# supranational/sppark

Hardware: AMD Instinct MI355X
Metric: MSM points/sec (BLS12-381 G1, 2^26 points) (higher is better)
Workload: dtype u32

## Files before the change

### sppark_amd/csrc/msm/msm_driver.hpp

```cpp
#pragma once
#include "msm_kernels.hpp"
#include "msm_coop_kernels.hpp"
#include "msm_plan.hpp"
#include "../ec/jacobian_host.hpp"
#include "../util/runtime.hpp"
#include <algorithm>
#include <cmath>
#include <map>
#include <mutex>
#include <vector>

namespace sppark_amd {

template<class FD, class FH, class FRp>
class msm_t {
public:
    typedef FD fp_d;
    static constexpr bool G2_COOP_BUILT = field_is_internal<FD>::value && !field_is_montx<FD>::value;
    typedef mont_dev<FRp> fr_d;
    typedef FH fp_h;
    typedef typename xyzz_dev<fp_d>::mem_t bucket_t;
    typedef jacobian_host<fp_h> point_t;
    static constexpr int STD_WORDS = sizeof(FH) / 4;
    static constexpr size_t FP_BYTES = sizeof(FH);
// ... 248 lines not shown
    {
        if (tune.wbits) return std::min(26u, std::max(8u, tune.wbits));
        unsigned w = 0; double best = 0;
        for (unsigned c = 8; c <= 26; c++) {
            const double cost = (double)((FRp::NBITS - 1) / c + 1) * (double)np + 3.0 * (double)((size_t)1 << (c - 1));
            if (w == 0 || cost < best) { best = cost; w = c; }
        }
        return w;
    }
    void preload(const void* points, size_t np, size_t ffi_affine_sz, bool fixed_base = false)
    {
        HIP_OK(hipSetDevice(gpu->hip_id));
        HIP_OK(hipStreamSynchronize(stream));
        join_default_stream();
        if (np != 0 && (points == nullptr || ffi_affine_sz < 2 * FP_BYTES || np > (1u << 31))) HIP_OK(hipErrorInvalidValue);
        if (np != 0 && fixed_base && !MONTX) HIP_OK(hipErrorNotSupported);
        if (np != 0 && fixed_base && (tune.wbits || np >= FIXED_BASE_MIN)
            && (size_t)((FRp::NBITS - 1) / fixed_base_width(np) + 1) * np >= ((size_t)1 << 31)) HIP_OK(hipErrorInvalidValue);
        if (pre_points) { HIP_OK(hipFree(pre_points)); pre_points = nullptr; pre_n = pre_stride = 0; }
        pre_fb_wbits = pre_fb_nwins = 0;
        if (np == 0) return;
        if (fixed_base && !MONTX) HIP_OK(hipErrorNotSupported);
        if (fixed_base && !tune.wbits && np < FIXED_BASE_MIN) fixed_base = false;
        unsigned fb_w = 0, fb_nw = 1;
        if (fixed_base) {
            fb_w = fixed_base_width(np);
            fb_nw = (FRp::NBITS - 1) / fb_w + 1;
            fb_w = FRp::NBITS / fb_nw + (FRp::NBITS % fb_nw ? 1 : 0);
            if ((size_t)fb_nw * np >= ((size_t)1 << 31)) HIP_OK(hipErrorInvalidValue);
        }
        if (points == nullptr || ffi_affine_sz < 2 * FP_BYTES || np > (1u << 31)) HIP_OK(hipErrorInvalidValue);
        struct dev_buf {
            unsigned char* p = nullptr;
            ~dev_buf() { if (p) (void)hipFree(p); }
        } staging;
        try {
            if constexpr (INTERNAL) {
                const unsigned char* src = (const unsigned char*)points;
                if (!is_device_pointer(points)) {
                    HIP_OK(hipMalloc((void**)&staging.p, np * ffi_affine_sz));
                    HIP_OK(hipMemcpyAsync(staging.p, points, np * ffi_affine_sz, hipMemcpyHostToDevice, stream));
                    src = staging.p;
                }
                HIP_OK(dev_scratch_pool::malloc_or_drain((void**)&pre_points, (size_t)fb_nw * np * conv_stride()));
                launch_convert(pre_points, src, (unsigned)np, ffi_affine_sz);
                if constexpr (MONTX) if (fixed_base) {
                    hipLaunchKernelGGL(k_fixed_base_table<fp_d>, dim3((unsigned)((np + 255) / 256)), dim3(256), 0, stream,
                                       pre_points, (unsigned)np, fb_nw, (unsigned)FRp::NBITS);
                    HIP_OK(hipGetLastError());
                }
            } else {
                HIP_OK(hipMalloc((void**)&pre_points, np * ffi_affine_sz));
                HIP_OK(hipMemcpyAsync(pre_points, points, np * ffi_affine_sz,
                                      is_device_pointer(points) ? hipMemcpyDeviceToDevice : hipMemcpyHostToDevice, stream));
            }
            HIP_OK(hipStreamSynchronize(stream));
        } catch (...) {
            if (pre_points) { (void)hipFree(pre_points); pre_points = nullptr; }
            throw;
        }
        pre_n = np; pre_stride = ffi_affine_sz;
        if (fixed_base) { pre_fb_wbits = fb_w; pre_fb_nwins = fb_nw; }
    }
    unsigned fixed_base_windows() const { return pre_fb_nwins; }
    size_t preloaded() const { return pre_n; }

private:
    void launch_convert(unsigned char* dst, const unsigned char* src, unsigned n, size_t stride, hipStream_t on = nullptr)
    {
        if constexpr (INTERNAL) {
            if (on == nullptr) on = stream;
            unsigned grid = (n + 255) / 256;
            if constexpr (MONTX) {
                if ((stride == 2 * FP_BYTES || stride == 2 * FP_BYTES + 8) && ((size_t)src & 15) == 0 && tune.join != 6) {
                    if (stride == 2 * FP_BYTES) hipLaunchKernelGGL((k_convert_points_staged<fp_d, false>), dim3(grid), dim3(256), 0, on, dst, src, n);
                    else                        hipLaunchKernelGGL((k_convert_points_staged<fp_d, true>), dim3(grid), dim3(256), 0, on, dst, src, n);
                    HIP_OK(hipGetLastError());
                    return;
                }
            }
            if (stride > 2 * FP_BYTES) hipLaunchKernelGGL((k_convert_points<fp_d, true>), dim3(grid), dim3(256), 0, on, dst, src, n, (unsigned)stride);
            else                       hipLaunchKernelGGL((k_convert_points<fp_d, false>), dim3(grid), dim3(256), 0, on, dst, src, n, (unsigned)stride);
            HIP_OK(hipGetLastError());
        }
    }

    size_t choose_chunk(size_t n, size_t stage_per_point) const
    {
        size_t chunk = n;
        if (tune.chunk) chunk = std::min(n, std::max<size_t>(tune.chunk, 1));
        else if (stage_per_point && n > ((size_t)1 << 21)) {
            chunk = std::min<size_t>(std::max<size_t>(n / 4, (size_t)1 << 20), (size_t)1 << 24);
        }
        auto need = [&](size_t c) {
            return make_layout(make_plan(c, FRp::NBITS, tune), true).total + 2 * c * stage_per_point + 1024;
        };
        size_t limit = tune.max_scratch;
        if (!limit) {
            const bool blob_ok = make_layout(make_plan(chunk, FRp::NBITS, tune), true).total <= blob_sz;
            const bool stage_ok = stage_per_point == 0 || 2 * (chunk * stage_per_point + 512) <= stage_sz;
            if (blob_ok && stage_ok) return chunk;
            size_t free_b = 0, total_b = 0;
            if (hipMemGetInfo(&free_b, &total_b) != hipSuccess) { (void)hipGetLastError(); return chunk; }
            limit = free_b - (free_b >> 5) + blob_sz + stage_sz;
        }
        while (need(chunk) > limit && chunk > 4096) chunk = (chunk + 1) / 2;
        return chunk;
    }

    std::vector<size_t> chunk_bounds(size_t n, size_t chunk) const
    {
        std::vector<size_t> b{0};
        for (size_t lo = chunk; lo < n; lo += chunk) b.push_back(lo);
        b.push_back(n);
        return b;
    }

    void sort_group(hipStream_t ss, const msm_plan& p, const layout& l, unsigned b, unsigned w0, unsigned wn,
                    const u32* d_scalars, bool mont, unsigned fb_n = 0, unsigned fb_nwins = 0)
    {
        u32* digits = (u32*)(blob + l.digits[b]);
        u32* sorted = (u32*)(blob + l.sorted[b]);
        u32* H = (u32*)(blob + l.H[b]);
        u32* tot = (u32*)(blob + l.tot[b]);
        u32* off = (u32*)(blob + l.off[b]);
        void* partA = blob + l.partA[b];
        u32* offA = (u32*)(blob + l.offA[b]);
        const bool packed = p.IB != 0;
        unsigned ngp = 1; while (ngp < p.NG) ngp <<= 1;
        const partA_fmt fmt{H, p.IB, p.SH, ngp, p.nslabs};
        const unsigned nlong = p.nbits % p.nwins, sf = nlong == 0 ? wn : (nlong > w0 ? std::min(wn, nlong - w0) : 0u);
        if (fb_n) {
            unsigned grid = std::min<unsigned>((fb_n + 255) / 256, 256 * 16);
            hipLaunchKernelGGL(k_breakdown<fr_d>, dim3(grid), dim3(256), 0, ss,
                               digits, d_scalars, fb_n, fb_nwins, (unsigned)FRp::NBITS, (int)mont, 0u, fb_nwins);
        } else {
            unsigned grid = std::min<unsigned>((p.n + 255) / 256, 256 * 16);
            hipLaunchKernelGGL(k_breakdown<fr_d>, dim3(grid), dim3(256), 0, ss,
                               digits, d_scalars, p.n, p.nwins, p.nbits, (int)mont, w0, wn);
        }
        HIP_OK(hipGetLastError());
        size_t ldsA = (size_t)p.NA * 4, ldsB = ((size_t)1 << p.LB) * 4 + SORT_NT * 4 + (size_t)SORTB_STAGE * 4 + PARTA_MAX_GROUPS * 4;
        if (ldsA > 65536) { lds_attr((const void*)k_histA, ldsA); lds_attr(packed ? (const void*)k_scatterA<true> : (const void*)k_scatterA<false>, ldsA); }
        if (ldsB > 65536) lds_attr(packed ? (const void*)k_sortB<true> : (const void*)k_sortB<false>, ldsB);
        hipLaunchKernelGGL(k_histA, dim3(p.nslabs, wn), dim3(SORT_NT), ldsA, ss,
                           H, digits, p.n, p.nslabs, p.slab_sz, p.NA, p.LB, sf);
        HIP_OK(hipGetLastError());
        size_t na_total = (size_t)wn * p.NA;
        hipLaunchKernelGGL(k_scan_slabs, dim3((unsigned)((na_total + 255) / 256)), dim3(256), 0, ss,
                           H, tot, p.nslabs, p.NA, wn);
        HIP_OK(hipGetLastError());
        hipLaunchKernelGGL(k_scan_parts, dim3(wn), dim3(1024), 0, ss, offA, tot, p.NA);
        HIP_OK(hipGetLastError());
        if (p.NA <= SCATA_MAX_NA && p.LB < 16) {
            const size_t ldsS = scatterA_staged_lds(p.NA);
            lds_attr(packed ? (const void*)k_scatterA_staged<true> : (const void*)k_scatterA_staged<false>, ldsS);
            if (packed) hipLaunchKernelGGL(k_scatterA_staged<true>, dim3(p.nslabs, wn), dim3(SORT_NT), ldsS, ss,
                                           (u32*)partA, digits, H, offA, p.n, p.nslabs, p.slab_sz, p.NA, p.LB, sf, p.IB);
            else        hipLaunchKernelGGL(k_scatterA_staged<false>, dim3(p.nslabs, wn), dim3(SORT_NT), ldsS, ss,
                                           (uint2*)partA, digits, H, offA, p.n, p.nslabs, p.slab_sz, p.NA, p.LB, sf, p.IB);
        } else {
            if (packed) hipLaunchKernelGGL(k_scatterA<true>, dim3(p.nslabs, wn), dim3(SORT_NT), ldsA, ss,
                                           (u32*)partA, digits, H, offA, p.n, p.nslabs, p.slab_sz, p.NA, p.LB, sf, p.IB);
            else        hipLaunchKernelGGL(k_scatterA<false>, dim3(p.nslabs, wn), dim3(SORT_NT), ldsA, ss,
                                           (uint2*)partA, digits, H, offA, p.n, p.nslabs, p.slab_sz, p.NA, p.LB, sf, p.IB);
        }
        HIP_OK(hipGetLastError());
        const unsigned big = tune.big ? tune.big : p.big ? p.big : (1u << 18);
        u32* nbig = (u32*)(blob + l.bigl[b]); u32* blist = nbig + 1; u32* curB = (u32*)(blob + l.curB[b]);
        const bool may_be_big = p.n > big;
        if (may_be_big) HIP_OK(hipMemsetAsync(nbig, 0, 4, ss));
        if (packed) hipLaunchKernelGGL(k_sortB<true>, dim3(p.NA, wn), dim3(SORT_NT), ldsB, ss,
                                       sorted, off, (const u32*)partA, offA, p.n, p.NA, p.LB, sf, big, fmt);
        else        hipLaunchKernelGGL(k_sortB<false>, dim3(p.NA, wn), dim3(SORT_NT), ldsB, ss,
                                       sorted, off, (const uint2*)partA, offA, p.n, p.NA, p.LB, sf, big, fmt);
        HIP_OK(hipGetLastError());
        if (!may_be_big) return;
        hipLaunchKernelGGL(k_big_find, dim3((p.NA * wn + 255) / 256), dim3(256), 0, ss,
                           nbig, blist, off, offA, p.NA, p.LB, sf, wn, big);
        size_t ldsBig = ((size_t)1 << p.LB) * 4;
        const size_t avg = (size_t)p.n / p.NA;
        const unsigned split = avg > big / 2 ? (unsigned)std::min<size_t>(SORTB_SPLIT, avg / (BIG_STAGE / 2) + 1) : SORTB_SPLIT;
        if (packed) hipLaunchKernelGGL(k_big_hist<true>, dim3(1024), dim3(1024), ldsBig, ss, off, (const u32*)partA, offA, nbig, blist, p.n, p.NA, p.LB, sf, split);
        else        hipLaunchKernelGGL(k_big_hist<false>, dim3(1024), dim3(1024), ldsBig, ss, off, (const uint2*)partA, offA, nbig, blist, p.n, p.NA, p.LB, sf, split);
        hipLaunchKernelGGL(k_big_scan, dim3(p.NA > 64 && avg > big / 2 ? 1024 : 64), dim3(1024), 0, ss, off, curB, offA, nbig, blist, p.NA, p.LB, sf);
        const size_t ldsSc = big_scatter_lds(p.LB);
        if (ldsSc > 65536) lds_attr(packed ? (const void*)k_big_scatter<true> : (const void*)k_big_scatter<false>, ldsSc);
        if (packed) hipLaunchKernelGGL(k_big_scatter<true>, dim3(1024), dim3(1024), ldsSc, ss, sorted, curB, (const u32*)partA, offA, nbig, blist, p.n, p.NA, p.LB, sf, split, fmt);
        else        hipLaunchKernelGGL(k_big_scatter<false>, dim3(1024), dim3(1024), ldsSc, ss, sorted, curB, (const uint2*)partA, offA, nbig, blist, p.n, p.NA, p.LB, sf, split, fmt);
        HIP_OK(hipGetLastError());
    }

    void enqueue(const msm_plan& p, const layout& l, const unsigned char* d_points, size_t stride, bool preconverted,
                 const u32* d_scalars, bool mont, std_bucket_t* h_out, bool first_timed, unsigned fb_n = 0, unsigned fb_nwins = 0,
                 bool redo = false, bool may_defer = false)
    {
        const bool flagged = !preconverted && stride > 2 * FP_BYTES;
        const bool multi = p.G > 1;
        if (multi) need_aux();
        if (timing && first_timed && !redo) { need_tev(2 + 2 * p.G); HIP_OK(hipEventRecord(tev[0], stream)); }
        if (multi) {
            HIP_OK(hipEventRecord(ev_fork, stream));
            HIP_OK(hipStreamWaitEvent(aux, ev_fork, 0));
        }
        bucket_t* buckets = (bucket_t*)(blob + l.buckets);
        u32* keyA = (u32*)(blob + l.keyA); bucket_t* ptA = (bucket_t*)(blob + l.ptA);
        u32* keyB = (u32*)(blob + l.keyB); bucket_t* ptB = (bucket_t*)(blob + l.ptB);
        if (multi && !redo) HIP_OK(hipMemsetAsync(buckets, 0, (size_t)p.nwins * p.NB * sizeof(bucket_t), stream));

        for (unsigned g = 0; g < p.G && !redo; g++, gseq++) {
            const unsigned b = multi ? (gseq & 1) : 0, w0 = g * p.wpg, wn = std::min(p.wpg, p.nwins - w0);
            if (g == 0) {
                sort_group(stream, p, l, b, w0, wn, d_scalars, mont, fb_n, fb_nwins);
                if (INTERNAL && !preconverted) {
                    launch_convert(blob + l.conv, d_points, p.n, stride);
                    d_points = blob + l.conv;
                }
            } else {
                if (gseq >= 2) HIP_OK(hipStreamWaitEvent(aux, ev_accdone[b], 0));
                sort_group(aux, p, l, b, w0, wn, d_scalars, mont);
                HIP_OK(hipEventRecord(ev_sorted[b], aux));
                HIP_OK(hipStreamWaitEvent(stream, ev_sorted[b], 0));
            }
            if (timing && first_timed) HIP_OK(hipEventRecord(tev[2 + 2 * g], stream));
            {
                const u32* sorted = (const u32*)(blob + l.sorted[b]);
                const u32* off = (const u32*)(blob + l.off[b]);
                dim3 grid((p.chunks_per_win + 255) / 256, wn);
                bool by_pairs = false;
                if constexpr (G2_COOP_BUILT) {
                    if (tune.g2_coop == 1 || (tune.g2_coop == 0 && fp_d::NL >= 14)) {
                        by_pairs = true;
                        dim3 grid2((p.chunks_per_win + 63) / 64, wn);
                        hipLaunchKernelGGL((k_accumulate_g2c<fp_d>), grid2, dim3(G2C_NT), 0, stream,
                                           buckets, keyA, ptA, d_points, (unsigned)stride, sorted, off,
                                           p.n, p.NB, p.L, p.chunks_per_win, w0);
                    }
                }
                if (by_pairs) {}
                else if (flagged)
                    hipLaunchKernelGGL((k_accumulate<fp_d, true>), grid, dim3(256), 0, stream,
                                       buckets, keyA, ptA, d_points, (unsigned)stride, sorted, off,
                                       p.n, p.NB, p.L, p.chunks_per_win, w0);
                else
                    hipLaunchKernelGGL((k_accumulate<fp_d, false>), grid, dim3(256), 0, stream,
                                       buckets, keyA, ptA, d_points, (unsigned)stride, sorted, off,
                                       p.n, p.NB, p.L, p.chunks_per_win, w0);
                HIP_OK(hipGetLastError());
            }
            if (timing && first_timed) HIP_OK(hipEventRecord(tev[3 + 2 * g], stream));
            if (multi) HIP_OK(hipEventRecord(ev_accdone[b], stream));
        }

        const unsigned piece_cm = may_defer ? piece_tree_cmax(p, multi, fb_n) : 0;
        piece_pending = false;
        bool small_sums = false;
        if constexpr (MONTX)
            small_sums = !multi && fb_n == 0 && p.NB <= SMALL_SUMS_MAX_NB && p.NB >= 2 && tune.K1 == 0 && tune.top == 0 && tune.K == 0
                         && tune.join != 3 && tune.join != 4;
        bool flag_with_sums = false;
        if constexpr (MONTX) flag_with_sums = small_sums && (piece_cm != 0 || redo);
        if (flag_with_sums && !d_pflag) {
            HIP_OK(hipMalloc((void**)&d_pflag, 64));
            HIP_OK(hipMemsetAsync(d_pflag, 0, 64, stream));
        }
        if (piece_cm && !redo) {
            u32* flag = flag_with_sums ? d_pflag : (u32*)(blob + l.flag);
            if (!flag_with_sums) HIP_OK(hipMemsetAsync(flag, 0, 4, stream));
            const u32* off = (const u32*)(blob + l.off[0]);
            unsigned t_fused = ~0u;
            if constexpr (MONTX) if (tune.join != 4 && tune.join != 8)
                t_fused = piece_tail_t0((size_t)p.nwins * p.NB, piece_cm, tune.join >= 16 ? (size_t)1 << (tune.join - 16) : PIECE_FUSE_MAX);
            for (unsigned t = 0; (piece_cm >> (t + 1)) >= 1; t++) {
                const unsigned last = (piece_cm >> (t + 2)) == 0;
                const size_t nthr = (size_t)p.nwins * p.NB * (piece_cm >> (t + 1));
                if constexpr (MONTX) if (t == t_fused) {
                    const unsigned lgGB = piece_tail_lgGB(piece_cm, t);
                    const size_t nwg = (((size_t)p.nwins * p.NB) + ((size_t)1 << lgGB) - 1) >> lgGB;
                    hipLaunchKernelGGL(k_piece_tail_coop<fp_d>, dim3((unsigned)nwg), dim3(COOP_NT), 0, stream,
                                       buckets, keyA, ptA, off, p.NB, p.L, p.chunks_per_win, p.nwins, piece_cm, t, lgGB, flag);
                    HIP_OK(hipGetLastError());
                    break;
                }
                bool coop = false;
                if constexpr (MONTX) coop = nthr <= COOP_LEVEL_MAX && tune.join != 4;
                if constexpr (MONTX) {
                    if (coop) hipLaunchKernelGGL(k_piece_level_coop<fp_d>, dim3((unsigned)((nthr + 63) / 64)), dim3(COOP_NT), 0, stream,
                                                 buckets, keyA, ptA, off, p.NB, p.L, p.chunks_per_win, p.nwins, piece_cm, t, last, flag);
                }
                if (!coop) hipLaunchKernelGGL(k_piece_level<fp_d>, dim3((unsigned)((nthr + 255) / 256)), dim3(256), 0, stream,
                                              buckets, keyA, ptA, off, p.NB, p.L, p.chunks_per_win, p.nwins, piece_cm, t, last, flag);
                HIP_OK(hipGetLastError());
            }
            if (!h_flag) HIP_OK(hipHostMalloc((void**)&h_flag, 64, hipHostMallocDefault));
            if (!flag_with_sums) HIP_OK(hipMemcpyAsync(h_flag, flag, 4, hipMemcpyDeviceToHost, stream));
            h_flag_cur = flag_with_sums ? reinterpret_cast<const u32*>(h_out + p.nwins) : h_flag;
            piece_pending = true;
        }
        if (!piece_pending) {
            size_t nrec = (size_t)2 * p.nwins * p.chunks_per_win;
            u32* ik = keyA; bucket_t* ip = ptA; u32* ok = keyB; bucket_t* op = ptB;
            const u32* skip = nullptr;
            if (tune.join != 1 && !redo && (size_t)p.n / p.NB <= (size_t)4 * p.L) {
                u32* keyC = (u32*)(blob + l.keyC); u32* flag = (u32*)(blob + l.flag);
                HIP_OK(hipMemsetAsync(flag, 0, 4, stream));
                const size_t nthr = nrec / 2 + 1;
                hipLaunchKernelGGL(k_join_runs<fp_d>, dim3((unsigned)((nthr + 255) / 256)), dim3(256), 0, stream,
                                   buckets, keyC, keyA, ptA, (unsigned)nrec, flag);
                HIP_OK(hipGetLastError());
                ik = keyC; skip = flag;
            }
            bool coop_tree = false;
            if constexpr (MONTX) coop_tree = tune.join != 4 && tune.join != 2;
// ... 381 lines not shown
```

### sppark_amd/csrc/msm/msm_sort_kernels.hpp

```cpp
#pragma once
#include "../ff/mont_dev.hpp"
#include "msm_sort_records.hpp"

namespace sppark_amd {

static constexpr unsigned SORT_NT = 1024;
#define SORT_VGPRS 32
static constexpr int SORTB_UNROLL = 4;
static constexpr int SORTB_PER = 18;
static constexpr unsigned SORTB_STAGE = SORTB_PER * SORT_NT;

__host__ __device__ inline unsigned window_lb(unsigned LB, unsigned w, unsigned short_from)
{   return (w >= short_from && LB) ? LB - 1 : LB;   }

SPPARK_DEVFN u32 block_scan_excl(u32 s, u32* wsum, u32* total)
{
    const unsigned lane = threadIdx.x & 63, wave = threadIdx.x >> 6;
    u32 incl = s;
    #pragma unroll
    for (int dlt = 1; dlt < 64; dlt <<= 1) { u32 v = __shfl_up(incl, dlt); if (lane >= (unsigned)dlt) incl += v; }
    if (lane == 63) wsum[wave] = incl;
    __syncthreads();
    u32 wv = lane < 16 ? wsum[lane] : 0, before = lane < wave ? wv : 0, tot = wv;
    #pragma unroll
    for (int m = 1; m < 16; m <<= 1) { before += __shfl_xor(before, m); tot += __shfl_xor(tot, m); }
    before = __shfl(before, 0); *total = __shfl(tot, 0);
    __syncthreads();
    return before + incl - s;
}

__global__ __launch_bounds__(SORT_NT) __attribute__((amdgpu_num_vgpr(SORT_VGPRS)))
void k_histA(u32* __restrict__ H, const u32* __restrict__ digits, unsigned n,
             unsigned nslabs, unsigned slab_sz, unsigned NA, unsigned LBL, unsigned short_from)
{
    extern __shared__ u32 lds_cnt[];
    const unsigned slab = blockIdx.x, w = blockIdx.y, LB = window_lb(LBL, w, short_from);
    for (unsigned b = threadIdx.x; b < NA; b += blockDim.x) lds_cnt[b] = 0;
    __syncthreads();

    const unsigned lo = slab * slab_sz, hi = min(n, lo + slab_sz);
    const u32* dig = digits + (size_t)w * n;
    for (unsigned i = lo + threadIdx.x; i < hi; i += 4 * blockDim.x) {
        u32 d[4];
        #pragma unroll
        for (int u = 0; u < 4; u++) { unsigned j = i + u * blockDim.x; d[u] = j < hi ? dig[j] : 0; }
        #pragma unroll
        for (int u = 0; u < 4; u++) if (d[u]) atomicAdd(&lds_cnt[((d[u] & 0x7fffffffu) - 1) >> LB], 1u);
    }
    __syncthreads();

    u32* out = H + ((size_t)w * nslabs + slab) * NA;
    for (unsigned b = threadIdx.x; b < NA; b += blockDim.x) out[b] = lds_cnt[b];
}

__global__ __launch_bounds__(256)
void k_scan_slabs(u32* __restrict__ H, u32* __restrict__ tot, unsigned nslabs, unsigned NA, unsigned nwins)
{
    const size_t id = (size_t)blockIdx.x * 256 + threadIdx.x;
    if (id >= (size_t)nwins * NA) return;
    const unsigned w = id / NA, b = id % NA;
    u32 run = 0;
    for (unsigned s = 0; s < nslabs; s++) {
        u32* p = H + ((size_t)w * nslabs + s) * NA + b;
        u32 t = *p; *p = run; run += t;
    }
    tot[id] = run;
}

__global__ __launch_bounds__(1024)
void k_scan_parts(u32* __restrict__ offA, const u32* __restrict__ tot, unsigned NA)
{
    __shared__ u32 part[1024];
    const unsigned w = blockIdx.x, tid = threadIdx.x;
    const unsigned per = (NA + 1023) / 1024;
    const unsigned lo = min(NA, tid * per), hi = min(NA, lo + per);
    const u32* t = tot + (size_t)w * NA;
    u32 sum = 0;
    for (unsigned b = lo; b < hi; b++) sum += t[b];
    part[tid] = sum;
    __syncthreads();
    for (unsigned d = 1; d < 1024; d <<= 1) {
        u32 v = tid >= d ? part[tid - d] : 0;
        __syncthreads();
        part[tid] += v;
        __syncthreads();
    }
    u32 run = part[tid] - sum;
    u32* o = offA + (size_t)w * (NA + 1);
    for (unsigned b = lo; b < hi; b++) { o[b] = run; run += t[b]; }
    if (tid == 1023) o[NA] = part[1023];
}

template<bool PK>
__global__ __launch_bounds__(SORT_NT) __attribute__((amdgpu_num_vgpr(SORT_VGPRS)))
void k_scatterA(typename recA<PK>::type* __restrict__ partA, const u32* __restrict__ digits,
                const u32* __restrict__ H, const u32* __restrict__ offA,
                unsigned n, unsigned nslabs, unsigned slab_sz, unsigned NA, unsigned LBL, unsigned short_from, unsigned IB)
{
    extern __shared__ u32 lds_cur[];
    const unsigned slab = blockIdx.x, w = blockIdx.y, LB = window_lb(LBL, w, short_from);
    const u32* h = H + ((size_t)w * nslabs + slab) * NA;
    const u32* o = offA + (size_t)w * (NA + 1);
    for (unsigned b = threadIdx.x; b < NA; b += blockDim.x) lds_cur[b] = h[b] + o[b];
    __syncthreads();

    const unsigned lo = slab * slab_sz, hi = min(n, lo + slab_sz);
    const u32* dig = digits + (size_t)w * n;
    typename recA<PK>::type* dst = partA + (size_t)w * n;
    const u32 lomask = (1u << LB) - 1;
    for (unsigned i = lo + threadIdx.x; i < hi; i += 4 * blockDim.x) {
        u32 d[4];
        #pragma unroll
        for (int u = 0; u < 4; u++) { unsigned j = i + u * blockDim.x; d[u] = j < hi ? dig[j] : 0; }
        #pragma unroll
        for (int u = 0; u < 4; u++) {
            if (d[u]) {
                u32 k = (d[u] & 0x7fffffffu) - 1;
                u32 pos = atomicAdd(&lds_cur[k >> LB], 1u);
                dst[pos] = recA<PK>::make((i + u * blockDim.x) | (d[u] & 0x80000000u), k & lomask, LBL, IB);
            }
        }
    }
}

static constexpr int SCATA_PER = 14;
static constexpr unsigned SCATA_TILE = SCATA_PER * SORT_NT;
static constexpr unsigned SCATA_MAX_NA = 4 * SORT_NT;
static inline size_t scatterA_staged_lds(unsigned NA) { return (size_t)NA * 8 + 64 + (size_t)SCATA_TILE * 8; }

SPPARK_DEVFN void wait_vmem()
{
#if defined(__HIP_DEVICE_COMPILE__)
    __builtin_amdgcn_s_waitcnt(0x0f70);
#endif
}
SPPARK_DEVFN void lds_barrier()
{
#if defined(__HIP_DEVICE_COMPILE__)
    asm volatile("s_waitcnt lgkmcnt(0)\n\ts_barrier" ::: "memory");
#endif
}

template<bool PK>
__global__ __launch_bounds__(SORT_NT)
void k_scatterA_staged(typename recA<PK>::type* __restrict__ partA, const u32* __restrict__ digits,
                       const u32* __restrict__ H, const u32* __restrict__ offA,
                       unsigned n, unsigned nslabs, unsigned slab_sz, unsigned NA, unsigned LBL, unsigned short_from, unsigned IB)
{
    extern __shared__ u32 lds_sa[];
    constexpr unsigned NT = SORT_NT;
    u32* cnt = lds_sa;
    u32* G = cnt + NA;
    u32* wsum = G + NA;
    uint2* stage = reinterpret_cast<uint2*>(wsum + 16);
    const unsigned slab = blockIdx.x, w = blockIdx.y, tid = threadIdx.x, lane = tid & 63, wave = tid >> 6;
    const unsigned LB = window_lb(LBL, w, short_from);
    const u32* h = H + ((size_t)w * nslabs + slab) * NA;
    const u32* o = offA + (size_t)w * (NA + 1);
    u32 cur[4];
    #pragma unroll
    for (int i = 0; i < 4; i++) { unsigned b = 4 * tid + i; cur[i] = b < NA ? h[b] + o[b] : 0; if (b < NA) cnt[b] = 0; }

    const unsigned lo = slab * slab_sz, hi = min(n, lo + slab_sz);
    const u32* dig = digits + (size_t)w * n;
    typename recA<PK>::type* dst = partA + (size_t)w * n;
    const u32 lomask = (1u << LB) - 1;
    u32 d[SCATA_PER], dn[SCATA_PER];
    #pragma unroll
    for (int u = 0; u < SCATA_PER; u++) { unsigned j = lo + u * NT + tid; dn[u] = j < hi ? dig[j] : 0; }
    __syncthreads();

    wait_vmem();
    #pragma unroll
    for (int u = 0; u < SCATA_PER; u++) d[u] = dn[u];
    for (unsigned t0 = lo; t0 < hi; t0 += SCATA_TILE) {
        #pragma unroll
        for (int u = 0; u < SCATA_PER; u++) { unsigned j = t0 + SCATA_TILE + u * NT + tid; dn[u] = j < hi ? dig[j] : 0; }
        #pragma unroll
        for (int u = 0; u < SCATA_PER; u++) if (d[u]) atomicAdd(&cnt[((d[u] & 0x7fffffffu) - 1) >> LB], 1u);
        lds_barrier();
        u32 c[4], s = 0;
        #pragma unroll
        for (int i = 0; i < 4; i++) { unsigned b = 4 * tid + i; c[i] = b < NA ? cnt[b] : 0; s += c[i]; }
        u32 incl = s;
        #pragma unroll
        for (int dlt = 1; dlt < 64; dlt <<= 1) { u32 v = __shfl_up(incl, dlt); if (lane >= (unsigned)dlt) incl += v; }
        if (lane == 63) wsum[wave] = incl;
        lds_barrier();
        u32 wv = lane < 16 ? wsum[lane] : 0, before = lane < wave ? wv : 0, total = wv;
        #pragma unroll
        for (int m = 1; m < 16; m <<= 1) { before += __shfl_xor(before, m); total += __shfl_xor(total, m); }
        before = __shfl(before, 0); total = __shfl(total, 0);
        u32 run = before + incl - s;
        #pragma unroll
        for (int i = 0; i < 4; i++) {
            unsigned b = 4 * tid + i;
            if (b < NA) { cnt[b] = run; G[b] = cur[i] - run; }
            cur[i] += c[i]; run += c[i];
        }
        lds_barrier();
        #pragma unroll
        for (int u = 0; u < SCATA_PER; u++) {
            if (d[u]) {
                u32 k = (d[u] & 0x7fffffffu) - 1, p = k >> LB;
                u32 pos = atomicAdd(&cnt[p], 1u);
                stage[pos] = make_uint2((t0 + u * NT + tid) | (d[u] & 0x80000000u), (p << 16) | (k & lomask));
            }
        }
        lds_barrier();
        wait_vmem();
        #pragma unroll
        for (int u = 0; u < SCATA_PER; u++) d[u] = dn[u];
        #pragma unroll
        for (int i = 0; i < 4; i++) { unsigned b = 4 * tid + i; if (b < NA) cnt[b] = 0; }
        #pragma unroll
        for (int u = 0; u < SCATA_PER; u++) {
            unsigned e = u * NT + tid;
            if (e < total) { uint2 v = stage[e]; dst[G[v.y >> 16] + e] = recA<PK>::make(v.x, v.y & 0xffffu, LBL, IB); }
        }
        lds_barrier();
    }
}

template<bool PK>
__global__ __launch_bounds__(SORT_NT) __attribute__((amdgpu_num_vgpr(64)))
void k_sortB(u32* __restrict__ sorted, u32* __restrict__ off, const typename recA<PK>::type* __restrict__ partA,
             const u32* __restrict__ offA, unsigned n, unsigned NA, unsigned LBL, unsigned short_from, unsigned big, partA_fmt fmt)
{
    extern __shared__ u32 lds[];
    typedef typename recA<PK>::type rec_t;
    constexpr unsigned NT = SORT_NT;
    const unsigned LB = window_lb(LBL, blockIdx.y, short_from);
    const size_t NB = (size_t)NA << LBL;
    const unsigned NL = 1u << LB;
    const u32 kmask = (1u << LBL) - 1;
    u32* cnt = lds;
    u32* part = lds + NL;
    u32* stage = part + NT;
    u32* bnd = stage + SORTB_STAGE;
    const unsigned khi = blockIdx.x, w = blockIdx.y, tid = threadIdx.x;
    const u32* oA = offA + (size_t)w * (NA + 1);
    const unsigned begin = oA[khi], end = oA[khi + 1];
    const rec_t* src = partA + (size_t)w * n;
    if (end - begin > big) {
        if (khi == NA - 1 && tid == 0) off[(size_t)w * (NB + 1) + NB] = end;
        if (LB != LBL) for (unsigned b = tid; b < NL; b += NT) off[(size_t)w * (NB + 1) + ((size_t)(NA + khi) << LB) + b] = oA[NA];
        return;
    }
    if (LB != LBL) for (unsigned b = tid; b < NL; b += NT) off[(size_t)w * (NB + 1) + ((size_t)(NA + khi) << LB) + b] = oA[NA];

    const bool in_regs = end - begin <= SORTB_STAGE;
    rec_t rr[SORTB_PER];
    for (unsigned b = tid; b < NL; b += NT) cnt[b] = 0;
    if (PK) partA_bounds(bnd, fmt, w, khi, NA, tid);
    __syncthreads();
    if (in_regs) {
        #pragma unroll
        for (int u = 0; u < SORTB_PER; u++) {
            unsigned j = begin + tid + u * NT;
            if (j < end) rr[u] = src[j];
        }
        #pragma unroll
        for (int u = 0; u < SORTB_PER; u++) if (begin + tid + u * NT < end) atomicAdd(&cnt[recA<PK>::key(rr[u], kmask)], 1u);
    } else {
        for (unsigned i = begin + tid; i < end; i += SORTB_UNROLL * NT) {
            rec_t r[SORTB_UNROLL];
            #pragma unroll
            for (int u = 0; u < SORTB_UNROLL; u++) { unsigned j = i + u * NT; if (j < end) r[u] = src[j]; }
            #pragma unroll
            for (int u = 0; u < SORTB_UNROLL; u++) if (i + u * NT < end) atomicAdd(&cnt[recA<PK>::key(r[u], kmask)], 1u);
        }
    }
    __syncthreads();

    const unsigned per = (NL + NT - 1) / NT;
    const unsigned lo = min(NL, tid * per), hi = min(NL, lo + per);
    u32 sum = 0;
    #pragma unroll 1
    for (unsigned b = lo; b < hi; b++) sum += cnt[b];
    u32 all;
    u32 run = begin + block_scan_excl(sum, part, &all);
    u32* o = off + (size_t)w * (NB + 1) + ((size_t)khi << LB);
    #pragma unroll 1
    for (unsigned b = lo; b < hi; b++) { u32 c = cnt[b]; cnt[b] = run; o[b] = run; run += c; }
    if (khi == NA - 1 && tid == 0) off[(size_t)w * (NB + 1) + NB] = end;
    __syncthreads();

    u32* dst = sorted + (size_t)w * n;
    if (in_regs) {
        #pragma unroll
        for (int u = 0; u < SORTB_PER; u++)
            if (begin + tid + u * NT < end)
                stage[atomicAdd(&cnt[recA<PK>::key(rr[u], kmask)], 1u) - begin] = recA<PK>::entry(rr[u], tid + u * NT, LBL, fmt, bnd);
        __syncthreads();
        for (unsigned i = tid; i < end - begin; i += NT) dst[begin + i] = stage[i];
        return;
    }
    for (unsigned i = begin + tid; i < end; i += SORTB_UNROLL * NT) {
        rec_t r[SORTB_UNROLL];
        #pragma unroll
        for (int u = 0; u < SORTB_UNROLL; u++) { unsigned j = i + u * NT; if (j < end) r[u] = src[j]; }
        #pragma unroll
        for (int u = 0; u < SORTB_UNROLL; u++) {
            if (i + u * NT < end) {
                u32 pos = atomicAdd(&cnt[recA<PK>::key(r[u], kmask)], 1u);
                dst[pos] = recA<PK>::entry(r[u], i + u * NT - begin, LBL, fmt, bnd);
            }
        }
    }
}

static constexpr unsigned SORTB_SPLIT = 64;
static constexpr int BIG_UNROLL = 4;

__global__ __launch_bounds__(256)
void k_big_find(u32* __restrict__ nbig, u32* __restrict__ list, u32* __restrict__ off,
                const u32* __restrict__ offA, unsigned NA, unsigned LBL, unsigned short_from, unsigned nwins, unsigned big)
{
    const unsigned id = blockIdx.x * blockDim.x + threadIdx.x;
    bool listed = false;
    if (id < NA * nwins) {
        const unsigned w = id / NA, khi = id % NA;
        const u32* oA = offA + (size_t)w * (NA + 1);
        listed = oA[khi + 1] - oA[khi] > big;
        if (listed) list[atomicAdd(nbig, 1u)] = id;
    }
    unsigned long long m = __ballot(listed);
    while (m) {
        const unsigned l = __builtin_ctzll(m); m &= m - 1;
        const unsigned pid = (id & ~63u) + l, w = pid / NA, khi = pid % NA, LB = window_lb(LBL, w, short_from);
        u32* o = off + (size_t)w * (((size_t)NA << LBL) + 1) + ((size_t)khi << LB);
        for (unsigned j = threadIdx.x & 63; j < (1u << LB); j += 64) o[j] = 0;
    }
}

__device__ inline bool big_slice(const u32* nbig, const u32* list, const u32* offA, unsigned NA, unsigned item, unsigned split,
                                 unsigned& w, unsigned& khi, unsigned& lo, unsigned& hi, unsigned& begin)
{
    const unsigned b = item / split, s = item % split;
    if (b >= *nbig) return false;
    w = list[b] / NA; khi = list[b] % NA;
    const u32* oA = offA + (size_t)w * (NA + 1);
    begin = oA[khi];
    const unsigned end = oA[khi + 1];
    const unsigned per = (end - begin + split - 1) / split;
    lo = min(end, begin + s * per); hi = min(end, lo + per);
    return true;
}

template<bool PK>
__global__ __launch_bounds__(1024)
void k_big_hist(u32* __restrict__ off, const typename recA<PK>::type* __restrict__ partA, const u32* __restrict__ offA,
                const u32* __restrict__ nbig, const u32* __restrict__ list, unsigned n, unsigned NA, unsigned LBL, unsigned short_from,
                unsigned split)
{
    extern __shared__ u32 lds[];
    const unsigned tid = threadIdx.x;
    const u32 kmask = (1u << LBL) - 1;
    for (unsigned item = blockIdx.x; ; item += gridDim.x) {
        unsigned w, khi, lo, hi, begin;
        if (!big_slice(nbig, list, offA, NA, item, split, w, khi, lo, hi, begin)) return;
        const unsigned LB = window_lb(LBL, w, short_from), NL = 1u << LB;
        for (unsigned j = tid; j < NL; j += 1024) lds[j] = 0;
        __syncthreads();
        const typename recA<PK>::type* src = partA + (size_t)w * n;
        for (unsigned i = lo + tid; i < hi; i += BIG_UNROLL * 1024) {
            u32 k[BIG_UNROLL];
            #pragma unroll
            for (int u = 0; u < BIG_UNROLL; u++) { unsigned j = i + u * 1024; k[u] = j < hi ? recA<PK>::key(src[j], kmask) : 0xffffffffu; }
            #pragma unroll
            for (int u = 0; u < BIG_UNROLL; u++) if (k[u] != 0xffffffffu) atomicAdd(&lds[k[u]], 1u);
        }
// ... 118 lines not shown
```

### sppark_amd/csrc/msm/msm_sort_records.hpp

```cpp
#pragma once
#include "../ff/mont_dev.hpp"

namespace sppark_amd {

struct partA_fmt {
    const u32* H;
    unsigned IB, SH, NGP, nslabs;
};
static constexpr unsigned PARTA_MAX_GROUPS = 128;
template<bool PK> struct recA;
template<> struct recA<false> {
    typedef uint2 type;
    SPPARK_DEVFN static type make(u32 idx_sign, u32 k, unsigned, unsigned) { return make_uint2(idx_sign, k); }
    SPPARK_DEVFN static u32 key(const type& r, u32) { return r.y; }
    SPPARK_DEVFN static u32 entry(const type& r, unsigned, unsigned, const partA_fmt&, const u32*) { return r.x; }
};
template<> struct recA<true> {
    typedef u32 type;
    SPPARK_DEVFN static type make(u32 idx_sign, u32 k, unsigned LBL, unsigned IB)
    {   return (idx_sign & 0x80000000u) | ((idx_sign & ((1u << IB) - 1)) << LBL) | k;   }
    SPPARK_DEVFN static u32 key(const type& r, u32 kmask) { return r & kmask; }
    SPPARK_DEVFN static u32 entry(const type& r, unsigned q, unsigned LBL, const partA_fmt& f, const u32* bnd)
    {
        unsigned g = 0;
        for (unsigned s = f.NGP >> 1; s; s >>= 1) if (bnd[g + s] <= q) g += s;
        return (r & 0x80000000u) | (((r & 0x7fffffffu) >> LBL) + (g << f.IB));
    }
};
SPPARK_DEVFN void partA_bounds(u32* bnd, const partA_fmt& f, unsigned w, unsigned khi, unsigned NA, unsigned tid)
{
    if (tid < f.NGP) {
        const unsigned slab = tid << f.SH;
        bnd[tid] = tid == 0 ? 0u : slab < f.nslabs ? f.H[((size_t)w * f.nslabs + slab) * NA + khi] : 0xffffffffu;
    }
}

}
```

Baseline: 513.9 million.

## Stage final packed records in scatterA and locate bucket runs via bitmaps

Result: no change. 517.0 million, median of 6 (+0.6%).

```diff
diff --git a/sppark_amd/csrc/msm/msm_driver.hpp b/sppark_amd/csrc/msm/msm_driver.hpp
--- a/sppark_amd/csrc/msm/msm_driver.hpp
+++ b/sppark_amd/csrc/msm/msm_driver.hpp
@@ -424,13 +424,18 @@
         HIP_OK(hipGetLastError());
         hipLaunchKernelGGL(k_scan_parts, dim3(wn), dim3(1024), 0, ss, offA, tot, p.NA);
         HIP_OK(hipGetLastError());
-        if (p.NA <= SCATA_MAX_NA && p.LB < 16) {
-            const size_t ldsS = scatterA_staged_lds(p.NA);
-            lds_attr(packed ? (const void*)k_scatterA_staged<true> : (const void*)k_scatterA_staged<false>, ldsS);
-            if (packed) hipLaunchKernelGGL(k_scatterA_staged<true>, dim3(p.nslabs, wn), dim3(SORT_NT), ldsS, ss,
-                                           (u32*)partA, digits, H, offA, p.n, p.nslabs, p.slab_sz, p.NA, p.LB, sf, p.IB);
-            else        hipLaunchKernelGGL(k_scatterA_staged<false>, dim3(p.nslabs, wn), dim3(SORT_NT), ldsS, ss,
-                                           (uint2*)partA, digits, H, offA, p.n, p.nslabs, p.slab_sz, p.NA, p.LB, sf, p.IB);
+        if (p.NA <= SCATA_MAX_NA) {
+            if (packed) {
+                const size_t ldsS = scatterA_staged_lds<true>(p.NA);
+                lds_attr((const void*)k_scatterA_staged<true>, ldsS);
+                hipLaunchKernelGGL(k_scatterA_staged<true>, dim3(p.nslabs, wn), dim3(SORT_NT), ldsS, ss,
+                                   (u32*)partA, digits, H, offA, p.n, p.nslabs, p.slab_sz, p.NA, p.LB, sf, p.IB);
+            } else {
+                const size_t ldsS = scatterA_staged_lds<false>(p.NA);
+                lds_attr((const void*)k_scatterA_staged<false>, ldsS);
+                hipLaunchKernelGGL(k_scatterA_staged<false>, dim3(p.nslabs, wn), dim3(SORT_NT), ldsS, ss,
+                                   (uint2*)partA, digits, H, offA, p.n, p.nslabs, p.slab_sz, p.NA, p.LB, sf, p.IB);
+            }
         } else {
             if (packed) hipLaunchKernelGGL(k_scatterA<true>, dim3(p.nslabs, wn), dim3(SORT_NT), ldsA, ss,
                                            (u32*)partA, digits, H, offA, p.n, p.nslabs, p.slab_sz, p.NA, p.LB, sf, p.IB);
diff --git a/sppark_amd/csrc/msm/msm_sort_kernels.hpp b/sppark_amd/csrc/msm/msm_sort_kernels.hpp
--- a/sppark_amd/csrc/msm/msm_sort_kernels.hpp
+++ b/sppark_amd/csrc/msm/msm_sort_kernels.hpp
@@ -9,9 +9,6 @@
 static constexpr int SORTB_UNROLL = 4;
 static constexpr int SORTB_PER = 18;
 static constexpr unsigned SORTB_STAGE = SORTB_PER * SORT_NT;
-
-__host__ __device__ inline unsigned window_lb(unsigned LB, unsigned w, unsigned short_from)
-{   return (w >= short_from && LB) ? LB - 1 : LB;   }
 
 SPPARK_DEVFN u32 block_scan_excl(u32 s, u32* wsum, u32* total)
 {
@@ -123,10 +120,9 @@
     }
 }
 
-static constexpr int SCATA_PER = 14;
-static constexpr unsigned SCATA_TILE = SCATA_PER * SORT_NT;
+static_assert(SCATA_NT == SORT_NT, "the staged scatter runs in the sort kernels' work-group size");
 static constexpr unsigned SCATA_MAX_NA = 4 * SORT_NT;
-static inline size_t scatterA_staged_lds(unsigned NA) { return (size_t)NA * 8 + 64 + (size_t)SCATA_TILE * 8; }
+template<bool PK> static inline size_t scatterA_staged_lds(unsigned NA) { return scatA_tile<PK>::lds_bytes(NA); }
 
 SPPARK_DEVFN void wait_vmem()
 {
@@ -148,76 +144,57 @@
                        unsigned n, unsigned nslabs, unsigned slab_sz, unsigned NA, unsigned LBL, unsigned short_from, unsigned IB)
 {
     extern __shared__ u32 lds_sa[];
+    typedef scatA_tile<PK> T;
     constexpr unsigned NT = SORT_NT;
-    u32* cnt = lds_sa;
-    u32* G = cnt + NA;
-    u32* wsum = G + NA;
-    uint2* stage = reinterpret_cast<uint2*>(wsum + 16);
-    const unsigned slab = blockIdx.x, w = blockIdx.y, tid = threadIdx.x, lane = tid & 63, wave = tid >> 6;
-    const unsigned LB = window_lb(LBL, w, short_from);
+    constexpr int PER = T::PER;
+    const unsigned slab = blockIdx.x, w = blockIdx.y, tid = threadIdx.x;
+    T t;
+    t.NA = NA; t.LB = window_lb(LBL, w, short_from); t.LBL = LBL; t.IB = IB;
+    t.carve(lds_sa);
     const u32* h = H + ((size_t)w * nslabs + slab) * NA;
     const u32* o = offA + (size_t)w * (NA + 1);
     u32 cur[4];
     #pragma unroll
-    for (int i = 0; i < 4; i++) { unsigned b = 4 * tid + i; cur[i] = b < NA ? h[b] + o[b] : 0; if (b < NA) cnt[b] = 0; }
+    for (int i = 0; i < 4; i++) { unsigned b = 4 * tid + i; cur[i] = b < NA ? h[b] + o[b] : 0; if (b < NA) t.cnt[b] = 0; }
 
     const unsigned lo = slab * slab_sz, hi = min(n, lo + slab_sz);
     const u32* dig = digits + (size_t)w * n;
-    typename recA<PK>::type* dst = partA + (size_t)w * n;
-    const u32 lomask = (1u << LB) - 1;
-    u32 d[SCATA_PER], dn[SCATA_PER];
+    typename T::rec_t* dst = partA + (size_t)w * n;
+    u32 d[PER], dn[PER];
     #pragma unroll
-    for (int u = 0; u < SCATA_PER; u++) { unsigned j = lo + u * NT + tid; dn[u] = j < hi ? dig[j] : 0; }
+    for (int u = 0; u < PER; u++) { unsigned j = lo + u * NT + tid; dn[u] = j < hi ? dig[j] : 0; }
     __syncthreads();
 
     wait_vmem();
     #pragma unroll
-    for (int u = 0; u < SCATA_PER; u++) d[u] = dn[u];
-    for (unsigned t0 = lo; t0 < hi; t0 += SCATA_TILE) {
-        #pragma unroll
-        for (int u = 0; u < SCATA_PER; u++) { unsigned j = t0 + SCATA_TILE + u * NT + tid; dn[u] = j < hi ? dig[j] : 0; }
-        #pragma unroll
-        for (int u = 0; u < SCATA_PER; u++) if (d[u]) atomicAdd(&cnt[((d[u] & 0x7fffffffu) - 1) >> LB], 1u);
+    for (int u = 0; u < PER; u++) d[u] = dn[u];
+    for (unsigned t0 = lo; t0 < hi; t0 += T::TILE) {
+        unsigned tl = tid;
+        asm volatile("" : "+v"(tl));
+        const unsigned lane = tl & 63, wave = tl >> 6;
+        #pragma unroll
+        for (int u = 0; u < PER; u++) { unsigned j = t0 + T::TILE + u * NT + tl; dn[u] = j < hi ? dig[j] : 0; }
+        t.count(d, tl);
         lds_barrier();
-        u32 c[4], s = 0;
-        #pragma unroll
-        for (int i = 0; i < 4; i++) { unsigned b = 4 * tid + i; c[i] = b < NA ? cnt[b] : 0; s += c[i]; }
+        u32 c[4];
+        const u32 s = t.own_counts(c, tl);
         u32 incl = s;
         #pragma unroll
         for (int dlt = 1; dlt < 64; dlt <<= 1) { u32 v = __shfl_up(incl, dlt); if (lane >= (unsigned)dlt) incl += v; }
-        if (lane == 63) wsum[wave] = incl;
+        if (lane == 63) t.wsum[wave] = incl;
         lds_barrier();
-        u32 wv = lane < 16 ? wsum[lane] : 0, before = lane < wave ? wv : 0, total = wv;
+        u32 wv = lane < 16 ? t.wsum[lane] : 0, before = lane < wave ? wv : 0, total = wv;
         #pragma unroll
         for (int m = 1; m < 16; m <<= 1) { before += __shfl_xor(before, m); total += __shfl_xor(total, m); }
-        before = __shfl(before, 0); total = __shfl(total, 0);
-        u32 run = before + incl - s;
-        #pragma unroll
-        for (int i = 0; i < 4; i++) {
-            unsigned b = 4 * tid + i;
-            if (b < NA) { cnt[b] = run; G[b] = cur[i] - run; }
-            cur[i] += c[i]; run += c[i];
-        }
+        before = __shfl(before, 0); total = __shfl(total, 0) & 0xffffu;
+        t.publish(cur, c, before + incl - s, tl);
         lds_barrier();
-        #pragma unroll
-        for (int u = 0; u < SCATA_PER; u++) {
-            if (d[u]) {
-                u32 k = (d[u] & 0x7fffffffu) - 1, p = k >> LB;
-                u32 pos = atomicAdd(&cnt[p], 1u);
-                stage[pos] = make_uint2((t0 + u * NT + tid) | (d[u] & 0x80000000u), (p << 16) | (k & lomask));
-            }
-        }
+        t.place(d, t0, tl);
         lds_barrier();
         wait_vmem();
         #pragma unroll
-        for (int u = 0; u < SCATA_PER; u++) d[u] = dn[u];
-        #pragma unroll
-        for (int i = 0; i < 4; i++) { unsigned b = 4 * tid + i; if (b < NA) cnt[b] = 0; }
-        #pragma unroll
-        for (int u = 0; u < SCATA_PER; u++) {
-            unsigned e = u * NT + tid;
-            if (e < total) { uint2 v = stage[e]; dst[G[v.y >> 16] + e] = recA<PK>::make(v.x, v.y & 0xffffu, LBL, IB); }
-        }
+        for (int u = 0; u < PER; u++) d[u] = dn[u];
+        t.write_out(dst, total, tl);
         lds_barrier();
     }
 }
diff --git a/sppark_amd/csrc/msm/msm_sort_records.hpp b/sppark_amd/csrc/msm/msm_sort_records.hpp
--- a/sppark_amd/csrc/msm/msm_sort_records.hpp
+++ b/sppark_amd/csrc/msm/msm_sort_records.hpp
@@ -35,4 +35,107 @@
     }
 }
 
+__host__ __device__ inline unsigned window_lb(unsigned LB, unsigned w, unsigned short_from)
+{   return (w >= short_from && LB) ? LB - 1 : LB;   }
+
+
+static constexpr unsigned SCATA_NT = 1024;
+SPPARK_DEVFN u32 lds_add(u32* p, u32 v)
+{
+#if defined(__HIP_DEVICE_COMPILE__)
+    return atomicAdd(p, v);
+#else
+    const u32 o = *p; *p = o + v; return o;
+#endif
 }
+SPPARK_DEVFN void lds_or(u32* p, u32 v)
+{
+#if defined(__HIP_DEVICE_COMPILE__)
+    atomicOr(p, v);
+#else
+    *p |= v;
+#endif
+}
+SPPARK_DEVFN void scatA_sched_fence()
+{
+#if defined(__HIP_DEVICE_COMPILE__)
+    __builtin_amdgcn_sched_barrier(0);
+#endif
+}
+template<bool PK> struct scatA_tile {
+    typedef typename recA<PK>::type rec_t;
+    static constexpr int PER = PK ? 28 : 14;
+    static constexpr unsigned NT = SCATA_NT, TILE = PER * NT, NCH = TILE / 64;
+    static constexpr int GRP = 7;
+    static_assert(TILE < 65536, "the block scan carries the tile's record count in 16 bits");
+    u32 *cnt, *G, *wsum, *first, *bits;
+    rec_t* stage;
+    unsigned NA, LB, LBL, IB;
+    static size_t lds_bytes(unsigned NA) { return (size_t)NA * 8 + 64 + (size_t)NCH * 12 + (size_t)TILE * sizeof(rec_t); }
+    SPPARK_DEVFN void carve(u32* lds)
+    {   cnt = lds; G = cnt + NA; wsum = G + NA; first = wsum + 16; bits = first + NCH; stage = reinterpret_cast<rec_t*>(bits + 2 * NCH);   }
+    SPPARK_DEVFN unsigned part(u32 d) const { return ((d & 0x7fffffffu) - 1) >> LB; }
+
+    SPPARK_DEVFN void count(const u32 (&d)[PER], unsigned tid) const
+    {
+        for (unsigned j = tid; j < 2 * NCH; j += NT) bits[j] = 0;
+        #pragma unroll
+        for (int u = 0; u < PER; u++) if (d[u]) lds_add(&cnt[part(d[u])], 1u);
+    }
+    SPPARK_DEVFN u32 own_counts(u32 (&c)[4], unsigned tid) const
+    {
+        u32 s = 0;
+        #pragma unroll
+        for (int i = 0; i < 4; i++) { const unsigned b = 4 * tid + i; c[i] = b < NA ? cnt[b] : 0; s += c[i] + (c[i] ? 0x10000u : 0u); }
+        return s;
+    }
+    SPPARK_DEVFN void publish(u32 (&cur)[4], const u32 (&c)[4], u32 before, unsigned tid) const
+    {
+        u32 run = before & 0xffffu, r = before >> 16;
+        #pragma unroll
+        for (int i = 0; i < 4; i++) {
+            const unsigned b = 4 * tid + i;
+            if (b < NA) cnt[b] = run;
+            if (c[i]) {
+                G[r] = cur[i] - run;
+                lds_or(&bits[run >> 5], 1u << (run & 31));
+                for (unsigned j = (run + 63) >> 6; j <= (run + c[i] - 1) >> 6; j++) first[j] = r;
+                r++;
+            }
+            cur[i] += c[i]; run += c[i];
+        }
+    }
+    SPPARK_DEVFN void place(const u32 (&d)[PER], unsigned t0, unsigned tid) const
+    {
+        const u32 lomask = (1u << LB) - 1;
+        #pragma unroll
+        for (int u = 0; u < PER; u++) {
+            if (u % GRP == 0) scatA_sched_fence();
+            if (d[u]) {
+                const u32 k = (d[u] & 0x7fffffffu) - 1;
+                stage[lds_add(&cnt[k >> LB], 1u)] = recA<PK>::make((t0 + u * NT + tid) | (d[u] & 0x80000000u), k & lomask, LBL, IB);
+            }
+        }
+    }
+    SPPARK_DEVFN void write_out(rec_t* dst, unsigned total, unsigned tid) const
+    {
+        #pragma unroll
+        for (int i = 0; i < 4; i++) { const unsigned b = 4 * tid + i; if (b < NA) cnt[b] = 0; }
+        const unsigned l = tid & 63;
+        const u64 below = (~(u64)0 >> (63 - l)) & ~(u64)1;
+        const u32* bw = bits + 2 * (tid >> 6);
+        const u32* fw = first + (tid >> 6);
+        const rec_t* sw = stage + tid;
+        #pragma unroll
+        for (int u = 0; u < PER; u++) {
+            if (u % GRP == 0) scatA_sched_fence();
+            const unsigned e = u * NT + tid;
+            if (e < total) {
+                const u64 starts = ((u64)bw[u * (NT / 32) + 1] << 32 | bw[u * (NT / 32)]) & below;
+                dst[G[fw[u * (NT / 64)] + (unsigned)__builtin_popcountll(starts)] + e] = sw[u * NT];
+            }
+        }
+    }
+};
+
+}
```
